# pcubillos/pyratbay

Measured on AMD Instinct MI355X. Metric: spectra/sec (1e5 wavenumbers x 80 layers), higher is better.
Workload: dtype f64; 1 GPU; 1e5 wavenumbers x 80 layers, 1e5 synthetic lines, transit; nwave=100001, nlayers=80, nlines=100000, wnosamp=180, voigt_grid=nlor=100 ndop=50 extent=300 cutoff=25, voigt_table_bytes=1448022784, parallelism=single GPU, 2 independent spectra in flight on 2 HIP streams, ranks=1, priming_spectra_in_init=32

## Files before the change

### pyratbay_amd/csrc/pb_ext_gather.hip

```cpp
#include <algorithm>
#include <climits>
#include <cmath>
#include <type_traits>
#include <vector>

#include "pb_ext_plan.h"

using namespace pbx;

namespace {

template <int RS, int NW>
__global__ __launch_bounds__(NW * 64) void k_ext_resample(LblArgs a)
{
    constexpr int NT = NW * 64;
    constexpr int kTileRS = (NW / RS) * kWaveSpan;
    static_assert(NW % RS == 0, "wavefronts must divide evenly into record shares");
    __shared__ double s_k[NT];
    __shared__ unsigned s_off[NT];
    __shared__ unsigned s_win[NT];

    int tile, layer;
    decode_block(a, tile, layer);
    if (layer < 0 || (a.res_cap > 0 && a.ls_resident[layer]))
        return;
    if (a.tsplit && a.tsplit[((int64_t)tile * kTileRS) / a.ts_tile] != 0)
        return;
    const int row = blockIdx.y;
    const int lane = threadIdx.x & 63;
    const int wave = __builtin_amdgcn_readfirstlane(threadIdx.x >> 6);

    const int64_t t0 = a.wbegin + (int64_t)tile * kTileRS;
    const int64_t tend = min(t0 + kTileRS, a.wbegin + a.wcount);
    const int part = wave % RS;
    const int rlo = (wave / RS) * kWaveSpan;
    const int64_t recbase = (int64_t)layer * a.ngroups;
    const int rhi = (int)min((int64_t)rlo + kWaveSpan, tend - t0);

    const int ofactor = a.ls_ofactor[layer];
    const double kthresh =
        a.ethresh * __longlong_as_double((long long)a.kmax_bits[(int64_t)layer * a.nrows + row]);
    const int osamp = a.osamp;

    double acc[kChunks][kLaneSamples];
#pragma unroll
    for (int s = 0; s < kChunks; s++)
        acc[s][0] = acc[s][1] = 0.0;

    for (int iso = 0; iso < a.niso; iso++) {
        const int iext = a.isoiext[iso];
        if (iext < 0 || (a.add ? 0 : iext) != row)
            continue;
        const int64_t li = (int64_t)layer * a.niso + iso;
        const int ilor = a.li_ilor[li];
        const double alphad = a.li_alphad[li];
        const double dens = a.li_dens[li];
        int64_t reach = a.li_hmax[li];
        if (a.cutoff > 0.0)
            reach = min(reach, (int64_t)(a.cutoff / a.ownstep) + 2 * (int64_t)ofactor + 2);
        reach += osamp + ofactor;
        const int64_t seg0 = a.iso_gstart[iso], seg1 = a.iso_gstart[iso + 1];
        const int64_t g0 = lower_bound_i32(a.giown, seg0, seg1, t0 * osamp - reach);
        const int64_t g1 = lower_bound_i32(a.giown, seg0, seg1, (tend - 1) * osamp + reach + 1);
        if (g0 >= g1)
            continue;
        const double vmin = a.own0 + ((double)a.giown[g0] - 1.0) * a.ownstep;
        const int idop_lo = pb::nearest_index(a.doppler, alphad * vmin, 0, a.ndop - 1);
        const int64_t cell_lo = (int64_t)ilor * a.ndop + idop_lo;
        const int64_t base_idx = a.pm_base[cell_lo] - kTile;
        const double *base = a.pm + base_idx;

        for (int64_t gb = g0; gb < g1; gb += NT) {
            __syncthreads();
            {
                const int64_t g = gb + threadIdx.x;
                double k = 0.0;
                unsigned off = 0, win = 0;
                if (g < g1) {
                    int ulo, uhi, cell, phi, q;
                    if (a.tsplit) {
                        const Rec16 r = a.rec16[(int64_t)layer * a.rec_pitch + a.pos2ph[g]];
                        k = r.k;
                        ulo = r.ulo;
                        uhi = ulo + (int)(r.lc & 0xfffu);
                        cell = (int)(r.lc >> 12);
                        const int d = a.psize[cell] - a.giown[g];
                        q = floor_div_inv(d, a.inv_osamp);
                        phi = d - q * osamp;
                    } else {
                        const int64_t idx = recbase + g;
                        k = a.rec_k[idx];
                        ulo = a.rec_ulo[idx];
                        uhi = a.rec_uhi[idx];
                        cell = a.rec_cell[idx];
                        phi = a.rec_phi[idx];
                        q = a.rec_q[idx];
                    }
                    const int64_t lo = max((int64_t)ulo, t0);
                    const int64_t hi = min((int64_t)uhi, tend);
                    if (!(k < kthresh) && lo < hi) {
                        if (a.add)
                            k *= dens;
                        win = (unsigned)(lo - t0) | ((unsigned)(hi - t0) << 16);
                        off = (unsigned)(a.pm_base[cell] + (int64_t)phi * a.pm_stride[cell] + q +
                                         t0 - base_idx);
                        if (a.experiment == 1)
                            off = (unsigned)(kTile + (lo - t0));
                    } else {
                        k = 0.0;
                    }
                }
                s_k[threadIdx.x] = k;
                s_off[threadIdx.x] = off;
                s_win[threadIdx.x] = win;
            }
            __syncthreads();
            const int nrec = a.experiment == 2 ? 0 : (int)min((int64_t)NT, g1 - gb);
            for (int b = 0; b < nrec; b += 64) {
                const int e = (b + lane) & (NT - 1);
                const unsigned my_win = s_win[e];
                const bool mine = RS == 1 || (int)(((gb + b + lane) >> 6) & (RS - 1)) == part;
                const bool hit = mine && b + lane < nrec && (int)(my_win & 0xffff) < rhi &&
                                 (int)(my_win >> 16) > rlo;
                unsigned long long mask = __ballot(hit);
                const double my_k = s_k[e];
                const unsigned my_off = s_off[e];
                while (mask) {
                    int src[kRecs];
#pragma unroll
                    for (int r = 0; r < kRecs; r++) {
                        src[r] = mask ? __builtin_amdgcn_readfirstlane(__builtin_ctzll(mask))
                                      : -1;
                        mask &= mask - 1;
                    }
                    double2 v[kRecs][kChunks];
                    double kk[kRecs];
                    int lo[kRecs], hi[kRecs];
#pragma unroll
                    for (int r = 0; r < kRecs; r++) {
                        const int sl = src[r] < 0 ? src[0] : src[r];
                        kk[r] = bcast(my_k, sl);
                        const unsigned win = (unsigned)__builtin_amdgcn_readlane((int)my_win, sl);
                        const unsigned off = (unsigned)__builtin_amdgcn_readlane((int)my_off, sl);
                        lo[r] = (int)(win & 0xffff);
                        hi[r] = (int)(win >> 16);
                        if (src[r] < 0)
                            kk[r] = 0.0;
                        const double *tab = base + off;
#pragma unroll
                        for (int s = 0; s < kChunks; s++) {
                            const int j = rlo + s * kChunk + 2 * lane;
                            const int jc = min(max(j, lo[r] - 1), hi[r] - 1);
                            v[r][s] = *reinterpret_cast<const double2 *>(tab + jc);
                        }
                    }
#pragma unroll
                    for (int r = 0; r < kRecs; r++) {
                        const unsigned span = (unsigned)(hi[r] - lo[r]);
#pragma unroll
                        for (int s = 0; s < kChunks; s++) {
                            const int j = rlo + s * kChunk + 2 * lane;
                            acc[s][0] = fma((unsigned)(j - lo[r]) < span ? kk[r] : 0.0,
                                            v[r][s].x, acc[s][0]);
                            acc[s][1] = fma((unsigned)(j + 1 - lo[r]) < span ? kk[r] : 0.0,
                                            v[r][s].y, acc[s][1]);
                        }
                    }
                }
            }
        }
    }

    if (RS > 1) {
        __shared__ double s_acc[NT * kChunks * kLaneSamples];
        __syncthreads();
#pragma unroll
        for (int s = 0; s < kChunks; s++) {
            s_acc[(threadIdx.x * kChunks + s) * kLaneSamples + 0] = acc[s][0];
            s_acc[(threadIdx.x * kChunks + s) * kLaneSamples + 1] = acc[s][1];
        }
        __syncthreads();
        if (part != 0)
            return;
#pragma unroll
        for (int s = 0; s < kChunks; s++) {
            for (int q = 1; q < RS; q++) {
                const int t = threadIdx.x + q * 64;
                acc[s][0] += s_acc[(t * kChunks + s) * kLaneSamples + 0];
                acc[s][1] += s_acc[(t * kChunks + s) * kLaneSamples + 1];
            }
        }
    }
    double *dst = a.ext + ((int64_t)layer * a.nrows + row) * a.wcount + (t0 - a.wbegin);
#pragma unroll
    for (int s = 0; s < kChunks; s++) {
        const int j = rlo + s * kChunk + 2 * lane;
        if (j < rhi)
            dst[j] = acc[s][0];
        if (j + 1 < rhi)
            dst[j + 1] = acc[s][1];
    }
}


template <int NW, int S, bool kDma, int kProbe = 0, int kIssue = 0, int kRows = 1>
__global__ __launch_bounds__(NW * 64, 8) void k_ext_staged(LblArgs a)
{
    constexpr int kThreads = NW * 64;
    constexpr int kSub = NW * kStageSpan;
    constexpr int kT = S * kSub;
    constexpr int kRowRegs = (kStageRowMax + kThreads - 1) / kThreads;
    static_assert(kT < 65536, "window coordinates are packed in 16 bits");
    extern __shared__ __align__(16) unsigned char smem[];
    const int osamp = a.osamp;
    double *s_row = reinterpret_cast<double *>(smem);
    struct __align__(16) Rec {
        double k;
        int qoff;
        unsigned win;
    };
    const int rowspan = a.rowlds + kStagePad;
    constexpr int kNB = 2;
    Rec *s_rec = reinterpret_cast<Rec *>(s_row + kNB * rowspan + kStagePad);
    long long *s_src = reinterpret_cast<long long *>(s_rec + kThreads);
    unsigned long long *s_desc = reinterpret_cast<unsigned long long *>(s_src);
    unsigned long long *s_segmask =
        reinterpret_cast<unsigned long long *>(s_src + kThreads);
    unsigned *s_m = reinterpret_cast<unsigned *>(s_segmask + NW);
    unsigned *s_seg = s_m;
    long long *s_cbase = reinterpret_cast<long long *>(s_m + kThreads);
    int *s_csize = reinterpret_cast<int *>(s_cbase + a.ndop);
    int *s_cstride = s_csize + a.ndop;
    int *s_part = s_cstride + a.ndop;
    const int vmax = osamp * a.nch_max;
    int *s_cum = s_part + NW;
    int *s_phs = s_cum + (vmax + 1);

    int tile, layer, zsplit;
    {
        const int id = blockIdx.x;
        const int k = id >> 3;
        tile = k % a.ntiles;
        const int grp = k / a.ntiles;
        const int unit = grp * 8 + ((grp & 1) ? 7 - (id & 7) : (id & 7));
        if (a.unit_tab) {
            const int e = unit < a.nunits ? a.unit_tab[unit] : -1;
            layer = e < 0 ? -1 : e >> 8;
            zsplit = e & 0xff;
        } else {
            layer = a.nlayers - 1 - unit / a.nsplit;
            zsplit = unit % a.nsplit;
        }
    }
    if (layer < 0 || (a.res_cap > 0 && a.ls_resident[layer]) || (a.wave_cap > 0 && a.ls_wave[layer]))
        return;
    const int nsp = a.tsplit ? a.tsplit[tile] : a.lsplit ? a.lsplit[layer] : a.nsplit;
    if (zsplit >= nsp)
        return;
    const int row = blockIdx.y;
    const int tid = threadIdx.x;
    const int lane = tid & 63;
    const int wave = __builtin_amdgcn_readfirstlane(tid >> 6);
    unsigned long long pc[22] = {0, 0, 0, 0, 0, 0, 0, 0, 0, 0, 0, 0, 0, 0, 0, 0, 0, 0, 0, 0, 0, 0};
    auto tick = [&]() -> unsigned long long {
        if constexpr (kProbe == 4)
            return (unsigned long long)__builtin_amdgcn_s_memtime();
        return 0ull;
    };
    unsigned long long real_birth = 0;
    if constexpr (kProbe == 4) {
        real_birth = (unsigned long long)__builtin_amdgcn_s_memrealtime();
        const unsigned long long c0 = tick();
        const unsigned long long c1 = tick();
        const unsigned long long c2 = tick();
        pc[16] = (c2 - c0) + 0 * c1;
        pc[17] = 1;
    }
    const unsigned long long t_birth = tick();

    const int64_t t0 = a.wbegin + (int64_t)tile * kT;
    const int64_t tend = min(t0 + kT, a.wbegin + a.wcount);
    const int tlen = (int)(tend - t0);
    const int rlo = wave * kStageSpan;

    const double kthresh =
        a.ethresh * __longlong_as_double((long long)a.kmax_bits[(int64_t)layer * a.nrows + row]);
    const int64_t recbase = a.rec16 ? (int64_t)layer * a.rec_pitch - a.grp_lo
                                    : (int64_t)layer * a.ngroups;
    double *const out = zsplit == 0
                            ? a.ext
                            : a.part + (int64_t)(zsplit - 1) * a.nlayers * a.nrows * a.wcount;
    double *const dst = out + ((int64_t)layer * a.nrows + row) * a.wcount + (t0 - a.wbegin);

    double acc[S][4];
#pragma unroll
    for (int u = 0; u < S; u++)
        acc[u][0] = acc[u][1] = acc[u][2] = acc[u][3] = 0.0;
    if (a.accumulate) {
#pragma unroll
        for (int u = 0; u < S; u++)
#pragma unroll
            for (int c = 0; c < 4; c++) {
                const int j = rlo + u * kSub + c * 64 + lane;
                if (j < tlen)
                    acc[u][c] = dst[j];
            }
    }
    for (int i = tid; i < kNB * rowspan + kStagePad; i += kThreads)
        s_row[i] = 0.0;

    double ring[kDma ? 1 : 2 * kRowRegs];
    int rowlim = a.rowlds;
    constexpr bool kMulti = kDma && kIssue == 0 && kRows > 1;
    int pitch = rowspan, nrow = 1;
    static_assert(kRows <= kStageRowsMax && kStageRowsMax <= NW,
                  "a wavefront requests at most one row of a step");
    const unsigned row_lds0 = (unsigned)(size_t)(__attribute__((address_space(3))) char *)(
        reinterpret_cast<char *>(s_row + kStagePad));
    int npiece = (rowlim + 127) >> 7;
    typedef int dma_v4i __attribute__((ext_vector_type(4)));
#define PB_DMA_OPEN "s_mov_b32 %0, m0\n\ts_mov_b32 m0, %1\n\ts_nop 0\n\t"
#define PB_DMA_LD(off) "buffer_load_dwordx4 %2, %3, 0 offen offset:" #off " lds\n\t"
#define PB_DMA_LD1 PB_DMA_LD(0)
#define PB_DMA_LD2 PB_DMA_LD1 PB_DMA_LD(1024)
#define PB_DMA_LD3 PB_DMA_LD2 PB_DMA_LD(2048)
#define PB_DMA_LD4 PB_DMA_LD3 PB_DMA_LD(3072)
#define PB_DMA_GROUP(pad, loads, dst_, voff_)                                                    \
    do {                                                                                         \
        unsigned keep;                                                                           \
        asm volatile(pad PB_DMA_OPEN loads "s_mov_b32 m0, %0"                                    \
                     : "=&s"(keep)                                                               \
                     : "s"(dst_), "v"(voff_), "s"(rsrc)                                          \
                     : "memory");                                                                \
    } while (0)
    auto dma_pieces = [&](unsigned dst, int voff, dma_v4i rsrc) {
        const unsigned dst4 = dst + 4096;
        const int voff4 = voff + 4096;
        switch (npiece) {
        case 1: PB_DMA_GROUP("s_nop 4\n\t", PB_DMA_LD1, dst, voff); break;
        case 2: PB_DMA_GROUP("s_nop 4\n\t", PB_DMA_LD2, dst, voff); break;
        case 3: PB_DMA_GROUP("s_nop 4\n\t", PB_DMA_LD3, dst, voff); break;
        case 4: PB_DMA_GROUP("s_nop 4\n\t", PB_DMA_LD4, dst, voff); break;
        case 5:
            PB_DMA_GROUP("s_nop 4\n\t", PB_DMA_LD4, dst, voff);
            PB_DMA_GROUP("", PB_DMA_LD1, dst4, voff4);
            break;
        case 6:
            PB_DMA_GROUP("s_nop 4\n\t", PB_DMA_LD4, dst, voff);
            PB_DMA_GROUP("", PB_DMA_LD2, dst4, voff4);
            break;
        case 7:
            PB_DMA_GROUP("s_nop 4\n\t", PB_DMA_LD4, dst, voff);
            PB_DMA_GROUP("", PB_DMA_LD3, dst4, voff4);
            break;
        case 8:
            PB_DMA_GROUP("s_nop 4\n\t", PB_DMA_LD4, dst, voff);
            PB_DMA_GROUP("", PB_DMA_LD4, dst4, voff4);
            break;
        default: break;
        }
    };
#undef PB_DMA_GROUP
#undef PB_DMA_LD4
#undef PB_DMA_LD3
#undef PB_DMA_LD2
#undef PB_DMA_LD1
#undef PB_DMA_LD
#undef PB_DMA_OPEN
    auto dma_desc = [&](unsigned long long d, int buf, auto part, int c_lo, int c_hi,
                        unsigned long long tref = 0) {
        const unsigned dlo = (unsigned)__builtin_amdgcn_readfirstlane((int)d);
        const unsigned dhi = (unsigned)__builtin_amdgcn_readfirstlane((int)(d >> 32));
        const long long first = ((long long)(dhi & 0xffu) << 32) | dlo;
        const int len = (int)((dhi >> 8) & 0xfffu), mlo = (int)(dhi >> 20);
        const unsigned long long base = (unsigned long long)(a.pm + first);
        dma_v4i rsrc;
        rsrc.x = __builtin_amdgcn_readfirstlane((int)base);
        rsrc.y = __builtin_amdgcn_readfirstlane((int)((base >> 32) & 0xffffu));
        rsrc.z = __builtin_amdgcn_readfirstlane(len * 8);
        rsrc.w = 0x00020000;
        int voff = (2 * lane - (mlo & ~1)) * 8;
        unsigned dst = (unsigned)__builtin_amdgcn_readfirstlane((int)(row_lds0 + buf * (kMulti ? pitch : rowspan) * 8));
        if constexpr (kProbe == 4) {
            if (tref)
                pc[20] += tick() - tref;
        }
        if constexpr (!decltype(part)::value) {
            dma_pieces(dst, voff, rsrc);
        } else {
            voff += 1024 * c_lo;
            dst += 1024 * (unsigned)c_lo;
            for (int c = c_lo; c < c_hi && c * 128 < rowlim; c++) {
                unsigned keep;
                asm volatile("s_nop 4\n\t"
                             "s_mov_b32 %0, m0\n\t"
                             "s_mov_b32 m0, %1\n\t"
                             "s_nop 0\n\t"
                             "buffer_load_dwordx4 %2, %3, 0 offen lds\n\t"
                             "s_mov_b32 m0, %0"
                             : "=&s"(keep)
                             : "s"(dst), "v"(voff), "s"(rsrc)
                             : "memory");
                voff += 1024;
                dst += 1024;
            }
        }
    };
    auto dma_row = [&](int sg, int buf, unsigned long long tref = 0) {
        dma_desc(s_desc[sg], buf, std::false_type(), 0, 0, tref);
    };
    auto load_row = [&](int sg, auto Rc, double *reg) {
        constexpr int R = decltype(Rc)::value;
        const unsigned long long d = s_desc[sg];
        const unsigned dlo = (unsigned)__builtin_amdgcn_readfirstlane((int)d);
        const unsigned dhi = (unsigned)__builtin_amdgcn_readfirstlane((int)(d >> 32));
        const long long first = ((long long)(dhi & 0xffu) << 32) | dlo;
        const int len = (int)((dhi >> 8) & 0xfffu), mlo = (int)(dhi >> 20);
        const __amdgpu_buffer_rsrc_t rsrc = __builtin_amdgcn_make_buffer_rsrc(
            (void *)(a.pm + first), 0, len * 8, 0x00020000);
        typedef int v2i __attribute__((ext_vector_type(2)));
#pragma unroll
        for (int r = 0; r < R; r++) {
            const v2i v = __builtin_amdgcn_raw_buffer_load_b64(
                rsrc, (tid + r * kThreads - mlo) * 8, 0, 0);
            reg[r] = __hiloint2double(v.y, v.x);
        }
    };
    auto store_row = [&](int buf, auto Rc, const double *reg, auto Dc) {
        constexpr int R = decltype(Rc)::value;
        constexpr int kInFlight = (decltype(Dc)::value - 1) * R;
        __builtin_amdgcn_s_waitcnt((kInFlight & 0xf) | (0x7 << 4) | (0xf << 8) |
                                   ((kInFlight >> 4) << 14));
        double *dst = s_row + kStagePad + buf * rowspan;
#pragma unroll
        for (int r = 0; r < R; r++) {
            if (wave * 64 + r * kThreads >= rowlim)
                continue;
            const int mm = tid + r * kThreads;
            if (mm < a.rowlds)
                dst[mm] = reg[r];
        }
    };

    pc[14] += tick() - t_birth;
    for (int iso = 0; iso < a.niso; iso++) {
        const int iext = a.isoiext[iso];
        if (iext < 0 || (a.add ? 0 : iext) != row)
            continue;
        if ((iso + 1) * osamp <= a.key_lo || iso * osamp >= a.key_hi)
            continue;
        const unsigned long long t_iso = tick();
        const int64_t li = (int64_t)layer * a.niso + iso;
        const double dens = a.li_dens[li];
        int64_t reach = a.li_hmax[li];
        if (a.cutoff > 0.0)
            reach = min(reach, (int64_t)(a.cutoff / a.ownstep) + 2 * (int64_t)a.ls_ofactor[layer] + 2);
        reach += osamp + a.ls_ofactor[layer];
        const int64_t flo = t0 * osamp - reach, fhi = (tend - 1) * osamp + reach;

        __syncthreads();
        const int cell0 = a.li_ilor[li] * a.ndop;
        for (int d = tid; d < a.ndop; d += kThreads) {
            s_cbase[d] = a.pm_base[cell0 + d];
            s_csize[d] = a.psize[cell0 + d];
            s_cstride[d] = a.pm_stride[cell0 + d];
        }
        {
            const int lim = min(a.rowlds, a.li_rowmax[li]);
            if (lim != rowlim) {
                for (int i = tid; i < kNB * rowspan + kStagePad; i += kThreads)
                    s_row[i] = 0.0;
                rowlim = lim;
                npiece = (lim + 127) >> 7;
                if constexpr (kMulti) {
                    const StageSlots sl = stage_slots(a.rowlds, lim, min(kRows, a.rows_cap));
                    pitch = sl.pitch;
                    nrow = sl.rows;
                }
            }
        }
        const int nch = a.nch_max > 1
                            ? (min(a.rowcap, a.li_rowmax[li]) + kChunkRow - 1) / kChunkRow
                            : 1;
        const int nvirt = osamp * nch;
        const int per = (nvirt + kThreads - 1) / kThreads;
        int mine = 0;
        for (int r = 0; r < per; r++) {
            const int pv = tid * per + r;
            const int p = pv / nch, c = pv - p * nch;
            if (pv < nvirt && ((nsp > 1 && p * nsp / osamp != zsplit) ||
                               iso * osamp + p < a.key_lo || iso * osamp + p >= a.key_hi)) {
                s_phs[pv] = 0;
                s_cum[pv] = 0;
            } else if (pv < nvirt) {
                const int32_t *bin = a.ph_bin + ((int64_t)iso * osamp + p) * (a.ph_nbins + 1);
                const int64_t binw = (int64_t)kBinSamples * osamp;
                int64_t clo = flo, chi = fhi;
                if (a.nch_max > 1) {
                    const int64_t c0 = (int64_t)c * kChunkRow;
                    clo = max(clo, (t0 - c0 - kChunkRow - 1) * osamp + a.li_hlo[li]);
                    chi = min(chi, (tend - c0 + 1) * osamp + a.li_hhi[li]);
                    if (chi < clo)
                        chi = clo - 1;
                }
                const int b0 = (int)min((int64_t)a.ph_nbins - 1, max((int64_t)0, clo) / binw);
                const int b1 = (int)min((int64_t)a.ph_nbins - 1, max((int64_t)0, chi + 1) / binw);
                const int32_t l0 = bin[b0], h0 = bin[b0 + 1], l1 = bin[b1], h1 = bin[b1 + 1];
                int64_t s0, s1;
                lower_bound2_i32(a.ph_iown, l0, h0, clo, l1, h1, chi + 1, s0, s1);
                s_phs[pv] = (int)s0;
                s_cum[pv] = (int)(s1 - s0);
                mine += (int)(s1 - s0);
            }
        }
        int incl = mine;
#pragma unroll
        for (int d = 1; d < 64; d <<= 1) {
            const int up = __shfl_up(incl, d);
            if (lane >= d)
                incl += up;
        }
        if (lane == 63)
            s_part[wave] = incl;
        __syncthreads();
        int base = 0, total = 0;
        for (int w = 0; w < NW; w++) {
            const int pw = s_part[w];
            if (w < wave)
                base += pw;
            total += pw;
        }
        int run = base + incl - mine;
        for (int r = 0; r < per; r++) {
            const int pv = tid * per + r;
            if (pv < nvirt) {
                const int c = s_cum[pv];
                s_cum[pv] = run;
                run += c;
            }
        }
        if (tid == 0)
            s_cum[nvirt] = total;
        __syncthreads();
        pc[0] += tick() - t_iso;

        for (int x0 = 0; x0 < total; x0 += kThreads) {
            const int nrec = min(kThreads, total - x0);
            const unsigned long long t_batch = tick();
            pc[11] += 1;
            __syncthreads();
            long long src = -1;
            unsigned mwin = 0;
            {
                double k = 0.0;
                unsigned win = 0;
                int qoff = 0;
                const int x = x0 + tid;
                if (x < total) {
                    int plo = 0, pup = nvirt;
                    while (pup - plo > 1) {
                        const int mid = (plo + pup) >> 1;
                        if (s_cum[mid] <= x)
                            plo = mid;
                        else
                            pup = mid;
                    }
                    const int64_t entry = s_phs[plo] + (x - s_cum[plo]);
                    const int64_t gidx = entry;
                    int c0 = 0;
                    if (a.nch_max > 1)
                        c0 = (plo % nch) * kChunkRow;
                    const int64_t idx = recbase + entry;
                    int ulo, uhi, q, cell, phi;
                    if (a.rec16) {
                        const Rec16 r = a.rec16[idx];
                        k = r.k;
                        ulo = r.ulo;
                        const int lbits = a.nch_max > 1 ? kLongLenBits : 12;
                        uhi = ulo + (int)(r.lc & ((1u << lbits) - 1u));
                        cell = (int)(r.lc >> lbits);
                        const int d = s_csize[cell - cell0] - a.ph_iown[gidx];
                        q = floor_div_inv(d, a.inv_osamp);
                        phi = d - q * osamp;
                        if (a.nch_max > 1) {
                            const int wlo = max(ulo + q, c0), whi = min(uhi + q, c0 + kChunkRow);
                            if (whi > wlo) {
                                ulo = wlo - q;
                                uhi = whi - q;
                            } else {
                                uhi = ulo;
                            }
                        }
                        q -= c0;
                    } else {
                        k = a.rec_k[idx];
                        ulo = a.rec_ulo[idx];
                        uhi = a.rec_uhi[idx];
                        q = a.rec_q[idx];
                        cell = a.rec_cell[idx];
                        phi = a.rec_phi[idx];
                    }
                    const int lo = (int)(max((int64_t)ulo, t0) - t0);
                    const int hi = (int)(min((int64_t)uhi, tend) - t0);
                    if (!(k < kthresh) && lo < hi) {
                        if (a.add)
                            k *= dens;
                        win = (unsigned)lo | ((unsigned)hi << 16);
                        qoff = (int)(q + t0) * 8;
                        if (kDma)
                            qoff -= ((ulo + q) & 1) * 8;
                        src = s_cbase[cell - cell0] + (long long)phi * s_cstride[cell - cell0] + c0;
                        mwin = (unsigned)(ulo + q) | ((unsigned)(uhi + q) << 16);
                    } else {
                        k = 0.0;
                    }
                }
                s_rec[tid].k = k;
                s_rec[tid].qoff = qoff;
                s_rec[tid].win = win;
                s_src[tid] = src;
                s_m[tid] = mwin;
            }
            __syncthreads();
            const unsigned long long t_seg = tick();
            pc[1] += t_seg - t_batch;
            bool start = false;
            {
                if (tid < nrec)
                    start = tid == 0 || s_src[tid] != s_src[tid - 1] || s_m[tid] != s_m[tid - 1];
                const unsigned long long m = __ballot(start);
                if (lane == 0)
                    s_segmask[wave] = m;
            }
            const bool live = start && s_src[tid] >= 0;
            const unsigned long long livemask = __ballot(live);
            if (lane == 0)
                s_part[wave] = __builtin_popcountll(livemask);
            __syncthreads();
            int nseg = 0;
            {
                int before = 0;
                for (int w = 0; w < NW; w++) {
                    const int c = s_part[w];
                    if (w < wave)
                        before += c;
                    nseg += c;
                }
                if (live) {
                    int w = tid >> 6;
                    unsigned long long m = s_segmask[w] & ~((2ull << (tid & 63)) - 1ull);
                    int end = nrec;
                    for (;;) {
                        if (m) {
                            end = min(nrec, w * 64 + (int)__builtin_ctzll(m));
                            break;
                        }
                        if (++w >= NW)
                            break;
                        m = s_segmask[w];
                    }
                    const int pos = before + __builtin_popcountll(livemask & ((1ull << lane) - 1ull));
                    s_seg[pos] = (unsigned)tid | ((unsigned)end << 16);
                    const unsigned long long mlo = mwin & 0xffffu, mhi = mwin >> 16;
                    s_desc[pos] = (unsigned long long)(src + (long long)mlo) | ((mhi - mlo) << 40) |
                                  (mlo << 52);
                }
            }
            __syncthreads();
            pc[2] += tick() - t_seg;
            if (nseg == 0)
                continue;
            unsigned hits[S];
            auto find_hits = [&](int sg0) {
                const int sgl = sg0 + lane;
                const unsigned sd = sgl < nseg ? s_seg[sgl] : 0u;
                const int i0 = (int)(sd & 0xffff), i1 = (int)(sd >> 16);
#pragma unroll
                for (int u = 0; u < S; u++) {
                    const int slo = rlo + u * kSub;
                    int lo = i0, hi = i1;
                    while (lo < hi) {
                        const int mid = (lo + hi) >> 1;
                        if ((int)(s_rec[mid].win >> 16) > slo)
                            hi = mid;
                        else
                            lo = mid + 1;
                    }
                    const int first = lo;
                    hi = i1;
                    while (lo < hi) {
                        const int mid = (lo + hi) >> 1;
                        if ((int)(s_rec[mid].win & 0xffff) >= slo + kStageSpan)
                            hi = mid;
                        else
                            lo = mid + 1;
                    }
                    hits[u] = slo < tlen ? (unsigned)first | ((unsigned)(lo - first) << 16) : 0u;
                }
            };
            auto walk = [&](int sg, int buf) {
                if ((sg & 63) == 0) {
                    const unsigned long long tf = tick();
                    find_hits(sg);
                    pc[3] += tick() - tf;
                }
                bool any = false;
                const char *rowp = reinterpret_cast<const char *>(
                    s_row + kStagePad + buf * (kMulti ? pitch : rowspan) + rlo + lane);
#pragma unroll
                for (int u = 0; u < S; u++) {
                    const unsigned h = (unsigned)__builtin_amdgcn_readlane((int)hits[u], sg & 63);
                    if (h < 0x10000u)
                        continue;
                    if constexpr (kProbe == 4) {
                        pc[12] += h >> 16;
                        any = true;
                    }
                    const int first = (int)(h & 0xffff);
                    const int last = first + (int)(h >> 16);
                    const char *rs = rowp + (size_t)u * kSub * 8;
                    const double2 *recs = reinterpret_cast<const double2 *>(s_rec);
                    auto visit = [&](const double2 raw) {
                        const double k = raw.x;
                        const int qoff = __double2loint(raw.y);
                        if constexpr (kProbe == 1 || kProbe == 2) {
                            const char *base = reinterpret_cast<const char *>(s_row);
                            const int off = ((int)(rs - base) + (kProbe == 1 ? 3 : 1) * 8 * lane + qoff) & ~15;
                            const double2 v0 = *reinterpret_cast<const double2 *>(base + off);
                            const double2 v1 = *reinterpret_cast<const double2 *>(
                                base + off + (kProbe == 1 ? 16 : 1024));
                            acc[u][0] = fma(k, v0.x, acc[u][0]);
                            acc[u][1] = fma(k, v0.y, acc[u][1]);
                            acc[u][2] = fma(k, v1.x, acc[u][2]);
                            acc[u][3] = fma(k, v1.y, acc[u][3]);
                            return;
                        }
                        const double *p0 = reinterpret_cast<const double *>(rs + qoff);
                        const double a0 = p0[0], a1 = p0[64], a2 = p0[128], a3 = p0[192];
                        acc[u][0] = fma(k, a0, acc[u][0]);
                        acc[u][1] = fma(k, a1, acc[u][1]);
                        acc[u][2] = fma(k, a2, acc[u][2]);
                        acc[u][3] = fma(k, a3, acc[u][3]);
                    };
                    int r = first;
                    for (; r + 3 < last; r += 4) {
                        const double2 w0 = recs[r], w1 = recs[r + 1], w2 = recs[r + 2],
                                      w3 = recs[r + 3];
                        visit(w0);
                        visit(w1);
                        visit(w2);
                        visit(w3);
                    }
                    if constexpr (kProbe == 3) {
                        if (r < last) {
                            double2 cur = recs[r];
                            for (; r + 1 < last; r++) {
                                const double2 nxt = recs[r + 1];
                                visit(cur);
                                cur = nxt;
                            }
                            visit(cur);
                        }
                    } else {
                        for (; r < last; r++)
                            visit(recs[r]);
                    }
                }
                if constexpr (kProbe == 4)
                    pc[13] += any ? 1 : 0;
            };
            auto run = [&](auto Dc, auto Rc) {
                constexpr int D = decltype(Dc)::value, R = decltype(Rc)::value;
                static_assert(D == 2, "two register sets, two LDS buffers");
                load_row(0, Rc, ring);
                load_row(min(1, nseg - 1), Rc, ring + R);
                store_row(0, Rc, ring, Dc);
                __syncthreads();
                int sg = 0;
                for (; sg + 2 < nseg; sg += 2) {
                    load_row(sg + 2, Rc, ring);
                    walk(sg, 0);
                    store_row(1, Rc, ring + R, Dc);
                    __syncthreads();
                    load_row(min(sg + 3, nseg - 1), Rc, ring + R);
                    walk(sg + 1, 1);
                    store_row(0, Rc, ring, Dc);
                    __syncthreads();
                }
                walk(sg, 0);
                if (sg + 1 < nseg) {
                    store_row(1, Rc, ring + R, std::integral_constant<int, 1>());
                    __syncthreads();
                    walk(sg + 1, 1);
                }
            };
            if (kDma) {
                if constexpr (kIssue == 1) {
                    unsigned long long dn = s_desc[min(nseg - 1, wave == 0 ? NW : wave)];
                    if (wave == 0)
                        dma_row(0, 0);
                    __builtin_amdgcn_s_waitcnt(0x0f70);
                    __syncthreads();
                    for (int sg = 0; sg < nseg; sg++) {
                        if (sg + 1 < nseg && wave == ((sg + 1) & (NW - 1))) {
                            dma_desc(dn, (sg + 1) & 1, std::false_type(), 0, 0);
                            dn = s_desc[min(nseg - 1, sg + 1 + NW)];
                        }
                        walk(sg, sg & 1);
                        __builtin_amdgcn_s_waitcnt(0x0f70);
                        __syncthreads();
                    }
                    continue;
                }
                if constexpr (kIssue == 2) {
                    constexpr int kPer = (8 + NW - 1) / NW;
                    unsigned long long dn = s_desc[min(nseg - 1, 1)];
                    dma_desc(s_desc[0], 0, std::true_type(), wave * kPer, wave * kPer + kPer);
                    __builtin_amdgcn_s_waitcnt(0x0f70);
                    __syncthreads();
                    for (int sg = 0; sg < nseg; sg++) {
                        const unsigned long long dcur = dn;
                        dn = s_desc[min(nseg - 1, sg + 2)];
                        if (sg + 1 < nseg)
                            dma_desc(dcur, (sg + 1) & 1, std::true_type(), wave * kPer, wave * kPer + kPer);
                        walk(sg, sg & 1);
                        __builtin_amdgcn_s_waitcnt(0x0f70);
                        __syncthreads();
                    }
                    continue;
                }
                if constexpr (!kMulti) {
                    unsigned long long ta = tick();
                    if (wave == 0)
                        dma_row(0, 0);
                    __builtin_amdgcn_s_waitcnt(0x0f70);
                    __syncthreads();
                    if constexpr (kProbe == 4) {
                        const unsigned long long tb = tick();
                        pc[8] += tb - ta;
                        ta = tb;
                    }
                    for (int sg = 0; sg < nseg; sg++) {
                        if (sg + 1 < nseg && wave == ((sg + 1) & (NW - 1)))
                            dma_row(sg + 1, (sg + 1) & 1, ta);
                        if constexpr (kProbe == 4) {
                            const unsigned long long tb = tick();
                            if (sg + 1 < nseg && wave == ((sg + 1) & (NW - 1))) {
                                pc[4] += tb - ta;
                                pc[19] += 1;
                            } else {
                                pc[18] += tb - ta;
                            }
                            ta = tb;
                            const unsigned long long f0 = pc[3];
                            walk(sg, sg & 1);
                            const unsigned long long tc = tick();
                            pc[5] += (tc - ta) - (pc[3] - f0);
                            __builtin_amdgcn_s_waitcnt(0x0f70);
                            const unsigned long long td = tick();
                            pc[6] += td - tc;
                            __syncthreads();
                            ta = tick();
                            pc[7] += ta - td;
                            pc[10] += 1;
                            pc[21] += 1;
                            continue;
                        }
                        walk(sg, sg & 1);
                        __builtin_amdgcn_s_waitcnt(0x0f70);
                        __syncthreads();
                    }
                    continue;
                }
                auto step_end = [&](int s0) { return min(min(s0 + nrow, nseg), (s0 | 63) + 1); };
                auto request = [&](int s0, int s1, int slot0, unsigned long long tref) {
                    const int g = s0 + ((wave - s0) & (NW - 1));
                    if (g < s1)
                        dma_row(g, slot0 + (g - s0), tref);
                    return g < s1;
                };
                unsigned long long ta = tick();
                int sg = 0, se = step_end(0), half = 0;
                request(0, se, 0, 0);
                __builtin_amdgcn_s_waitcnt(0x0f70);
                __syncthreads();
                if constexpr (kProbe == 4) {
                    const unsigned long long tb = tick();
                    pc[8] += tb - ta;
                    ta = tb;
                }
                while (sg < nseg) {
                    const int sn = step_end(se);
                    const bool asked = request(se, sn, (half ^ 1) * nrow, ta);
                    if constexpr (kProbe == 4) {
                        const unsigned long long tb = tick();
                        if (asked) {
                            pc[4] += tb - ta;
                            pc[19] += 1;
                        } else {
                            pc[18] += tb - ta;
                        }
                        ta = tb;
                        const unsigned long long f0 = pc[3];
                        for (int g = sg; g < se; g++)
                            walk(g, half * nrow + (g - sg));
                        const unsigned long long tc = tick();
                        pc[5] += (tc - ta) - (pc[3] - f0);
                        __builtin_amdgcn_s_waitcnt(0x0f70);
                        const unsigned long long td = tick();
                        pc[6] += td - tc;
                        __syncthreads();
                        ta = tick();
                        pc[7] += ta - td;
                        pc[10] += 1;
                        pc[21] += (unsigned long long)(se - sg);
                    } else {
                        (void)asked;
                        for (int g = sg; g < se; g++)
                            walk(g, half * nrow + (g - sg));
                        __builtin_amdgcn_s_waitcnt(0x0f70);
                        __syncthreads();
                    }
                    sg = se;
                    se = sn;
                    half ^= 1;
                }
            } else if (nseg > 0) {
                run(std::integral_constant<int, 2>(), std::integral_constant<int, kRowRegs>());
            }
        }
    }

    const unsigned long long t_out = tick();
#pragma unroll
    for (int u = 0; u < S; u++) {
#pragma unroll
        for (int c = 0; c < 4; c++) {
            const int j = rlo + u * kSub + c * 64 + lane;
            if (j < tlen)
                dst[j] = acc[u][c];
        }
    }
    if constexpr (kProbe == 4) {
        const unsigned long long t_end = tick();
        pc[14] += t_end - t_out;
        pc[9] = t_end - t_birth;
        pc[15] = (unsigned long long)__builtin_amdgcn_s_memrealtime() - real_birth;
        if (lane == 0 && a.probe)
            for (int i = 0; i < 22; i++)
                atomicAdd(&a.probe[(int64_t)layer * 24 + i], pc[i]);
    }
}

__global__ __launch_bounds__(kResThreads) void k_ext_resident(LblArgs a)
{
    extern __shared__ __align__(16) unsigned char smem[];
    struct __align__(16) Rec {
        double k;
        int off;
        unsigned win;
    };
    double *s_prof = reinterpret_cast<double *>(smem);
    const int zslot = a.res_cap;
    Rec *s_rec = reinterpret_cast<Rec *>(s_prof + a.res_cap + 2);
    int *s_cell = reinterpret_cast<int *>(s_rec + kResThreads);
    int *s_part = s_cell + kResThreads;

    int tile, layer;
    decode_block(a, tile, layer);
    if (layer < 0 || !a.ls_resident[layer])
        return;
    const int row = blockIdx.y;
    const int tid = threadIdx.x;
    const int lane = tid & 63;
    const int wave = __builtin_amdgcn_readfirstlane(tid >> 6);

    const int64_t t0 = a.wbegin + (int64_t)tile * kResTile;
    const int64_t tend = min(t0 + kResTile, a.wbegin + a.wcount);
    const int tlen = (int)(tend - t0);
    const double kthresh =
        a.ethresh * __longlong_as_double((long long)a.kmax_bits[(int64_t)layer * a.nrows + row]);
    const int64_t recbase = (int64_t)layer * a.ngroups;
    const int osamp = a.osamp;
    const int ofactor = a.ls_ofactor[layer];

    double acc[kResStrips];
#pragma unroll
    for (int u = 0; u < kResStrips; u++)
        acc[u] = 0.0;
    if (tid == 0)
        s_prof[zslot] = 0.0;

    for (int iso = 0; iso < a.niso; iso++) {
        const int iext = a.isoiext[iso];
        if (iext < 0 || (a.add ? 0 : iext) != row)
            continue;
        const int64_t li = (int64_t)layer * a.niso + iso;
        const double dens = a.li_dens[li];
        int64_t reach = a.li_hmax[li];
        if (a.cutoff > 0.0)
            reach = min(reach, (int64_t)(a.cutoff / a.ownstep) + 2 * (int64_t)ofactor + 2);
        reach += osamp + ofactor;
        const int64_t rs = reach / osamp + 1;
        const int32_t *gs = a.gs_start + (int64_t)iso * (a.nwave + 1);
        const int64_t g0 = gs[max((int64_t)0, t0 - rs)];
        const int64_t g1 = gs[min((int64_t)a.nwave, tend + rs)];

        for (int64_t gb = g0; gb < g1; gb += kResThreads) {
            const int nrec = (int)min((int64_t)kResThreads, g1 - gb);
            __syncthreads();
            {
                double k = 0.0;
                unsigned win = 0;
                int off = 0, cell = -1;
                if (tid < nrec) {
                    const int64_t idx = recbase + gb + tid;
                    k = a.rec_k[idx];
                    const int ulo = a.rec_ulo[idx], uhi = a.rec_uhi[idx];
                    const int lo = (int)(max((int64_t)ulo, t0) - t0);
                    const int hi = (int)(min((int64_t)uhi, tend) - t0);
                    if (!(k < kthresh) && lo < hi) {
                        if (a.add)
                            k *= dens;
                        cell = a.rec_cell[idx];
                        win = (unsigned)lo | ((unsigned)(hi - lo) << 16);
                        off = 8 * (a.rec_phi[idx] * a.pm_stride[cell] + (int)(a.rec_q[idx] + t0));
                    } else {
                        k = 0.0;
                    }
                }
                s_rec[tid].k = k;
                s_rec[tid].off = off;
                s_rec[tid].win = win;
                s_cell[tid] = cell;
            }
            int cur = -1;
            for (;;) {
                __syncthreads();
                int c = s_cell[tid];
                c = c > cur ? c : INT_MAX;
#pragma unroll
                for (int d = 32; d >= 1; d >>= 1)
                    c = min(c, __shfl_xor(c, d));
                if (lane == 0)
                    s_part[wave] = c;
                __syncthreads();
                c = INT_MAX;
                for (int w = 0; w < kResWaves; w++)
                    c = min(c, s_part[w]);
                if (c == INT_MAX)
                    break;
                cur = c;
                {
                    const int n = a.pm_stride[cur] * osamp;
                    const double *src = a.pm + a.pm_base[cur];
                    for (int i = tid; i < n; i += kResThreads)
                        s_prof[i] = src[i];
                }
                __syncthreads();
                const double2 *recs = reinterpret_cast<const double2 *>(s_rec);
#pragma unroll
                for (int u = 0; u < kResStrips; u++) {
                    const int slo = (wave + u * kResWaves) * 64;
                    if (slo >= tlen)
                        continue;
                    int first = INT_MAX, last = -1;
                    for (int b = 0; b < nrec; b += 64) {
                        const int e = b + lane;
                        const unsigned w = s_rec[e].win;
                        const int wlo = (int)(w & 0xffff);
                        const bool hit = s_cell[e] == cur && wlo < slo + 64 &&
                                         wlo + (int)(w >> 16) > slo;
                        const unsigned long long m = __ballot(hit);
                        if (m) {
                            first = min(first, b + (int)__builtin_ctzll(m));
                            last = max(last, b + 63 - (int)__builtin_clzll(m));
                        }
                    }
                    first = __builtin_amdgcn_readfirstlane(first);
                    last = __builtin_amdgcn_readfirstlane(last);
                    const unsigned j = (unsigned)(slo + lane);
                    typedef __attribute__((address_space(3))) const double lds_double;
                    const unsigned prof0 = (unsigned)(uintptr_t)(
                        (__attribute__((address_space(3))) const char *)s_prof);
                    const unsigned j8 = prof0 + j * 8u, z8 = prof0 + (unsigned)zslot * 8u;
                    double sum = acc[u];
#pragma unroll 4
                    for (int r = first; r <= last; r++) {
                        const double2 raw = recs[r];
                        const unsigned w = (unsigned)__double2hiint(raw.y);
                        const bool in = j - (w & 0xffffu) < (w >> 16);
                        const unsigned at = in ? j8 + (unsigned)__double2loint(raw.y) : z8;
                        sum = fma(raw.x, *(lds_double *)(uintptr_t)at, sum);
                    }
                    acc[u] = sum;
                }
            }
        }
    }

    double *dst = a.ext + ((int64_t)layer * a.nrows + row) * a.wcount + (t0 - a.wbegin);
#pragma unroll
    for (int u = 0; u < kResStrips; u++) {
        const int j = (wave + u * kResWaves) * 64 + lane;
        if (j < tlen)
            dst[j] = acc[u];
    }
}

#ifdef PB_EXPERIMENTS
constexpr int kScatterPad = 64;

template <int C>
__device__ inline void scatter_walk(const LblArgs &a, double *s_tile, int layer, int row,
                                    int64_t t0, int64_t tend, double kthresh)
{
    typedef int v2i __attribute__((ext_vector_type(2)));
    typedef int v4i __attribute__((ext_vector_type(4)));
    const int lane = threadIdx.x;
    const int osamp = a.osamp;
    const int ofactor = a.ls_ofactor[layer];
    const Rec32 *recs = a.rec32 + (int64_t)layer * a.ngroups;

    for (int iso = 0; iso < a.niso; iso++) {
        const int iext = a.isoiext[iso];
        if (iext < 0 || (a.add ? 0 : iext) != row)
            continue;
        const int64_t li = (int64_t)layer * a.niso + iso;
        const double dens = a.add ? a.li_dens[li] : 1.0;
        int64_t reach = a.li_hmax[li];
        if (a.cutoff > 0.0)
            reach = min(reach, (int64_t)(a.cutoff / a.ownstep) + 2 * (int64_t)ofactor + 2);
        reach += osamp + ofactor;
        const int64_t rs = reach / osamp + 1;
        const int32_t *gs = a.gs_start + (int64_t)iso * (a.nwave + 1);
        const int g0 = gs[max((int64_t)0, t0 - rs)];
        const int g1 = gs[min((int64_t)a.nwave, tend + rs)];

        v4i w0 = {0, 0, 0, 0}, w1 = {0, 0, 0, 0};
        auto fetch = [&](int g) {
            const v4i *p = reinterpret_cast<const v4i *>(recs + min(g + lane, g1 - 1));
            w0 = p[0];
            w1 = p[1];
        };
        if (g0 < g1)
            fetch(g0);
        for (int gb = g0; gb < g1; gb += 64) {
            const double kk = __hiloint2double(w0.y, w0.x);
            const long long off = ((long long)w0.w << 32) | (unsigned)w0.z;
            const int lo = max(w1.x, (int)t0), hi = min(w1.y, (int)tend);
            const bool ok = gb + lane < g1 && !(kk < kthresh) && lo < hi;
            const double b_k = kk * dens;
            const long long b_src = off + lo;
            const int b_lo = lo - (int)t0, b_n = hi - lo;
            unsigned long long live = __ballot(ok);
            if (gb + 64 < g1)
                fetch(gb + 64);

            struct Cur {
                int dst, nch;
                double k;
            };
            auto start = [&](double (&v)[C], Cur &c) {
                const int sl = (int)__builtin_ctzll(live);
                live &= live - 1;
                c.k = bcast(b_k, sl);
                const int s_lo = __builtin_amdgcn_readlane((int)b_src, sl);
                const int s_hi = __builtin_amdgcn_readlane((int)(b_src >> 32), sl);
                const int n = __builtin_amdgcn_readlane(b_n, sl);
                c.dst = __builtin_amdgcn_readlane(b_lo, sl);
                c.nch = (n + 63) >> 6;
                const __amdgpu_buffer_rsrc_t rsrc = __builtin_amdgcn_make_buffer_rsrc(
                    (void *)(a.pm + (((long long)s_hi << 32) | (unsigned)s_lo)), 0, n * 8,
                    0x00020000);
#pragma unroll
                for (int q = 0; q < C; q++) {
                    const v2i w = __builtin_amdgcn_raw_buffer_load_b64(rsrc, lane * 8, q * 512, 0);
                    v[q] = __hiloint2double(w.y, w.x);
                }
            };
            auto finish = [&](const double (&v)[C], const Cur &c) {
                double *dst = s_tile + c.dst + lane;
#pragma unroll
                for (int q = 0; q < C; q++)
                    if (q < c.nch)
                        __hip_atomic_fetch_add(dst + q * 64, c.k * v[q], __ATOMIC_RELAXED,
                                               __HIP_MEMORY_SCOPE_WORKGROUP);
            };
            double va[C], vb[C];
            Cur ca, cb;
            if (!live)
                continue;
            start(va, ca);
            for (;;) {
                if (!live) {
                    finish(va, ca);
                    break;
                }
                start(vb, cb);
                finish(va, ca);
                if (!live) {
                    finish(vb, cb);
                    break;
                }
                start(va, ca);
                finish(vb, cb);
            }
        }
    }
}

template <int T>
__global__ __launch_bounds__(64) void k_ext_scatter(LblArgs a)
{
    __shared__ double s_tile[T + kScatterPad];
    int tile, layer;
    decode_block(a, tile, layer);
    if (layer < 0)
        return;
    const int row = blockIdx.y;
    const int lane = threadIdx.x;
    const int64_t t0 = a.wbegin + (int64_t)tile * T;
    const int64_t tend = min(t0 + T, a.wbegin + a.wcount);
    const int tlen = (int)(tend - t0);
    const double kthresh =
        a.ethresh * __longlong_as_double((long long)a.kmax_bits[(int64_t)layer * a.nrows + row]);
    for (int i = lane; i < T + kScatterPad; i += 64)
        s_tile[i] = 0.0;
    const int rowmax = a.ls_block[layer] / a.osamp;
// ... 443 lines not shown
```

Baseline: 1188 spectra/s.

## Precompute LDS record offsets and uniform scalars to trim staged walk loop overhead

The hit word now holds an absolute LDS byte offset plus a count split into a multiple-of-four part and a remainder, so the inner record walk iterates over LDS pointers and handles the tail with fixed 1- and 2-record steps instead of index arithmetic. Buffer offsets are carried as running byte offsets toggled by XOR, and per-wave DMA ownership is tracked with an incrementing counter instead of modulo tests. Several wave-uniform values (threshold, density, cell base, pitch, row count) are forced into scalar registers with readfirstlane. The goal is less VALU/SALU bookkeeping in the hot gather loop, which adds a static limit on the LDS size and more intricate step scheduling.

```diff
diff --git a/pyratbay_amd/csrc/pb_ext_gather.hip b/pyratbay_amd/csrc/pb_ext_gather.hip
--- a/pyratbay_amd/csrc/pb_ext_gather.hip
+++ b/pyratbay_amd/csrc/pb_ext_gather.hip
@@ -222,6 +222,13 @@
     const int rowspan = a.rowlds + kStagePad;
     constexpr int kNB = 2;
     Rec *s_rec = reinterpret_cast<Rec *>(s_row + kNB * rowspan + kStagePad);
+    static_assert((kNB * (kStageRowMax + kStagePad) + kStagePad) * 8 + kThreads * 16 <= 65536,
+                  "a hit word holds the LDS offset of a record in 16 bits");
+    typedef double rec_v2 __attribute__((ext_vector_type(2)));
+    typedef const rec_v2 rec_cv2;
+    typedef __attribute__((address_space(3))) rec_cv2 *rec_lds_p;
+    const unsigned rec_off0 =
+        (unsigned)(size_t)(__attribute__((address_space(3))) char *)(reinterpret_cast<char *>(s_rec));
     long long *s_src = reinterpret_cast<long long *>(s_rec + kThreads);
     unsigned long long *s_desc = reinterpret_cast<unsigned long long *>(s_src);
     unsigned long long *s_segmask =
@@ -283,8 +290,12 @@
     const int tlen = (int)(tend - t0);
     const int rlo = wave * kStageSpan;
 
-    const double kthresh =
-        a.ethresh * __longlong_as_double((long long)a.kmax_bits[(int64_t)layer * a.nrows + row]);
+    auto uniform = [](double x) {
+        return __hiloint2double(__builtin_amdgcn_readfirstlane(__double2hiint(x)),
+                                __builtin_amdgcn_readfirstlane(__double2loint(x)));
+    };
+    const double kthresh = uniform(
+        a.ethresh * __longlong_as_double((long long)a.kmax_bits[(int64_t)layer * a.nrows + row]));
     const int64_t recbase = a.rec16 ? (int64_t)layer * a.rec_pitch - a.grp_lo
                                     : (int64_t)layer * a.ngroups;
     double *const out = zsplit == 0
@@ -367,7 +378,7 @@
 #undef PB_DMA_LD1
 #undef PB_DMA_LD
 #undef PB_DMA_OPEN
-    auto dma_desc = [&](unsigned long long d, int buf, auto part, int c_lo, int c_hi,
+    auto dma_desc = [&](unsigned long long d, unsigned boff, auto part, int c_lo, int c_hi,
                         unsigned long long tref = 0) {
         const unsigned dlo = (unsigned)__builtin_amdgcn_readfirstlane((int)d);
         const unsigned dhi = (unsigned)__builtin_amdgcn_readfirstlane((int)(d >> 32));
@@ -380,7 +391,7 @@
         rsrc.z = __builtin_amdgcn_readfirstlane(len * 8);
         rsrc.w = 0x00020000;
         int voff = (2 * lane - (mlo & ~1)) * 8;
-        unsigned dst = (unsigned)__builtin_amdgcn_readfirstlane((int)(row_lds0 + buf * (kMulti ? pitch : rowspan) * 8));
+        unsigned dst = (unsigned)__builtin_amdgcn_readfirstlane((int)(row_lds0 + boff));
         if constexpr (kProbe == 4) {
             if (tref)
                 pc[20] += tick() - tref;
@@ -406,8 +417,9 @@
             }
         }
     };
-    auto dma_row = [&](int sg, int buf, unsigned long long tref = 0) {
-        dma_desc(s_desc[sg], buf, std::false_type(), 0, 0, tref);
+    auto bufoff = [&](int buf) { return (unsigned)(buf * rowspan * 8); };
+    auto dma_row = [&](int sg, unsigned boff, unsigned long long tref = 0) {
+        dma_desc(s_desc[sg], boff, std::false_type(), 0, 0, tref);
     };
     auto load_row = [&](int sg, auto Rc, double *reg) {
         constexpr int R = decltype(Rc)::value;
@@ -451,7 +463,7 @@
             continue;
         const unsigned long long t_iso = tick();
         const int64_t li = (int64_t)layer * a.niso + iso;
-        const double dens = a.li_dens[li];
+        const double dens = uniform(a.li_dens[li]);
         int64_t reach = a.li_hmax[li];
         if (a.cutoff > 0.0)
             reach = min(reach, (int64_t)(a.cutoff / a.ownstep) + 2 * (int64_t)a.ls_ofactor[layer] + 2);
@@ -459,7 +471,7 @@
         const int64_t flo = t0 * osamp - reach, fhi = (tend - 1) * osamp + reach;
 
         __syncthreads();
-        const int cell0 = a.li_ilor[li] * a.ndop;
+        const int cell0 = __builtin_amdgcn_readfirstlane(a.li_ilor[li] * a.ndop);
         for (int d = tid; d < a.ndop; d += kThreads) {
             s_cbase[d] = a.pm_base[cell0 + d];
             s_csize[d] = a.psize[cell0 + d];
@@ -474,8 +486,8 @@
                 npiece = (lim + 127) >> 7;
                 if constexpr (kMulti) {
                     const StageSlots sl = stage_slots(a.rowlds, lim, min(kRows, a.rows_cap));
-                    pitch = sl.pitch;
-                    nrow = sl.rows;
+                    pitch = __builtin_amdgcn_readfirstlane(sl.pitch);
+                    nrow = __builtin_amdgcn_readfirstlane(sl.rows);
                 }
             }
         }
@@ -695,32 +707,32 @@
                         else
                             lo = mid + 1;
                     }
-                    hits[u] = slo < tlen ? (unsigned)first | ((unsigned)(lo - first) << 16) : 0u;
+                    const unsigned n = (unsigned)(lo - first);
+                    hits[u] = slo < tlen && n
+                                  ? (rec_off0 + (unsigned)first * 16u) << 16 | (n & ~3u) << 4 | (n & 3u)
+                                  : 0u;
                 }
             };
-            auto walk = [&](int sg, int buf) {
-                if ((sg & 63) == 0) {
-                    const unsigned long long tf = tick();
-                    find_hits(sg);
-                    pc[3] += tick() - tf;
-                }
+            auto block_hits = [&](int sg) {
+                const unsigned long long tf = tick();
+                find_hits(sg);
+                pc[3] += tick() - tf;
+            };
+            auto walk_row = [&](int sg, const char *rowp) {
                 bool any = false;
-                const char *rowp = reinterpret_cast<const char *>(
-                    s_row + kStagePad + buf * (kMulti ? pitch : rowspan) + rlo + lane);
 #pragma unroll
                 for (int u = 0; u < S; u++) {
                     const unsigned h = (unsigned)__builtin_amdgcn_readlane((int)hits[u], sg & 63);
-                    if (h < 0x10000u)
+                    if (h == 0u)
                         continue;
                     if constexpr (kProbe == 4) {
-                        pc[12] += h >> 16;
+                        pc[12] += ((h & 0xffc0u) >> 4) + (h & 3u);
                         any = true;
                     }
-                    const int first = (int)(h & 0xffff);
-                    const int last = first + (int)(h >> 16);
                     const char *rs = rowp + (size_t)u * kSub * 8;
-                    const double2 *recs = reinterpret_cast<const double2 *>(s_rec);
-                    auto visit = [&](const double2 raw) {
+                    rec_lds_p recs = (rec_lds_p)(size_t)(h >> 16);
+                    const rec_lds_p trips_end = (rec_lds_p)(size_t)((h >> 16) + (h & 0xffc0u));
+                    auto visit = [&](const rec_v2 raw) {
                         const double k = raw.x;
                         const int qoff = __double2loint(raw.y);
                         if constexpr (kProbe == 1 || kProbe == 2) {
@@ -742,33 +754,45 @@
                         acc[u][2] = fma(k, a2, acc[u][2]);
                         acc[u][3] = fma(k, a3, acc[u][3]);
                     };
-                    int r = first;
-                    for (; r + 3 < last; r += 4) {
-                        const double2 w0 = recs[r], w1 = recs[r + 1], w2 = recs[r + 2],
-                                      w3 = recs[r + 3];
+                    for (; recs != trips_end; recs += 4) {
+                        const rec_v2 w0 = recs[0], w1 = recs[1], w2 = recs[2], w3 = recs[3];
                         visit(w0);
                         visit(w1);
                         visit(w2);
                         visit(w3);
                     }
+                    const int left = (int)(h & 3u);
                     if constexpr (kProbe == 3) {
-                        if (r < last) {
-                            double2 cur = recs[r];
-                            for (; r + 1 < last; r++) {
-                                const double2 nxt = recs[r + 1];
+                        if (left) {
+                            rec_v2 cur = recs[0];
+                            for (int r = 1; r < left; r++) {
+                                const rec_v2 nxt = recs[r];
                                 visit(cur);
                                 cur = nxt;
                             }
                             visit(cur);
                         }
                     } else {
-                        for (; r < last; r++)
-                            visit(recs[r]);
+                        if (left & 1) {
+                            visit(recs[0]);
+                            recs += 1;
+                        }
+                        if (left & 2) {
+                            const rec_v2 w0 = recs[0], w1 = recs[1];
+                            visit(w0);
+                            visit(w1);
+                        }
                     }
                 }
                 if constexpr (kProbe == 4)
                     pc[13] += any ? 1 : 0;
             };
+            auto walk = [&](int sg, int buf) {
+                if ((sg & 63) == 0)
+                    block_hits(sg);
+                walk_row(sg, reinterpret_cast<const char *>(s_row + kStagePad + buf * rowspan + rlo + lane));
+            };
+            (void)walk;
             auto run = [&](auto Dc, auto Rc) {
                 constexpr int D = decltype(Dc)::value, R = decltype(Rc)::value;
                 static_assert(D == 2, "two register sets, two LDS buffers");
@@ -803,7 +827,7 @@
                     __syncthreads();
                     for (int sg = 0; sg < nseg; sg++) {
                         if (sg + 1 < nseg && wave == ((sg + 1) & (NW - 1))) {
-                            dma_desc(dn, (sg + 1) & 1, std::false_type(), 0, 0);
+                            dma_desc(dn, bufoff((sg + 1) & 1), std::false_type(), 0, 0);
                             dn = s_desc[min(nseg - 1, sg + 1 + NW)];
                         }
                         walk(sg, sg & 1);
@@ -822,7 +846,7 @@
                         const unsigned long long dcur = dn;
                         dn = s_desc[min(nseg - 1, sg + 2)];
                         if (sg + 1 < nseg)
-                            dma_desc(dcur, (sg + 1) & 1, std::true_type(), wave * kPer, wave * kPer + kPer);
+                            dma_desc(dcur, bufoff((sg + 1) & 1), std::true_type(), wave * kPer, wave * kPer + kPer);
                         walk(sg, sg & 1);
                         __builtin_amdgcn_s_waitcnt(0x0f70);
                         __syncthreads();
@@ -830,6 +854,10 @@
                     continue;
                 }
                 if constexpr (!kMulti) {
+                    const unsigned flip8 = (unsigned)rowspan * 8u;
+                    const char *const lane_row = reinterpret_cast<const char *>(s_row + kStagePad + rlo + lane);
+                    unsigned cur8 = 0;
+                    int mine = wave == 0 ? NW : wave;
                     unsigned long long ta = tick();
                     if (wave == 0)
                         dma_row(0, 0);
@@ -840,9 +868,12 @@
                         pc[8] += tb - ta;
                         ta = tb;
                     }
-                    for (int sg = 0; sg < nseg; sg++) {
-                        if (sg + 1 < nseg && wave == ((sg + 1) & (NW - 1)))
-                            dma_row(sg + 1, (sg + 1) & 1, ta);
+                    for (int sg = 0; sg < nseg; sg++, cur8 ^= flip8) {
+                        if (mine == sg + 1) {
+                            if (mine < nseg)
+                                dma_row(mine, cur8 ^ flip8, ta);
+                            mine += NW;
+                        }
                         if constexpr (kProbe == 4) {
                             const unsigned long long tb = tick();
                             if (sg + 1 < nseg && wave == ((sg + 1) & (NW - 1))) {
@@ -853,7 +884,9 @@
                             }
                             ta = tb;
                             const unsigned long long f0 = pc[3];
-                            walk(sg, sg & 1);
+                            if ((sg & 63) == 0)
+                                block_hits(sg);
+                            walk_row(sg, lane_row + cur8);
                             const unsigned long long tc = tick();
                             pc[5] += (tc - ta) - (pc[3] - f0);
                             __builtin_amdgcn_s_waitcnt(0x0f70);
@@ -866,21 +899,42 @@
                             pc[21] += 1;
                             continue;
                         }
-                        walk(sg, sg & 1);
+                        if ((sg & 63) == 0)
+                            block_hits(sg);
+                        walk_row(sg, lane_row + cur8);
                         __builtin_amdgcn_s_waitcnt(0x0f70);
                         __syncthreads();
                     }
                     continue;
                 }
-                auto step_end = [&](int s0) { return min(min(s0 + nrow, nseg), (s0 | 63) + 1); };
-                auto request = [&](int s0, int s1, int slot0, unsigned long long tref) {
-                    const int g = s0 + ((wave - s0) & (NW - 1));
-                    if (g < s1)
-                        dma_row(g, slot0 + (g - s0), tref);
-                    return g < s1;
+                constexpr bool kAligned = kRows <= 2;
+                const unsigned pitch8 = (unsigned)pitch * 8u, flip8 = (unsigned)nrow * pitch8;
+                const char *const lane_row = reinterpret_cast<const char *>(s_row + kStagePad + rlo + lane);
+                int mine = wave;
+                auto request = [&](int s0, int s1, unsigned boff0, unsigned long long tref) {
+                    const bool ask = mine < s1;
+                    if (ask) {
+                        dma_row(mine, boff0 + (unsigned)(mine - s0) * pitch8, tref);
+                        mine += NW;
+                    }
+                    return ask;
                 };
                 unsigned long long ta = tick();
-                int sg = 0, se = step_end(0), half = 0;
+                int bend = kAligned ? nseg : min(64, nseg);
+                int sg = 0, se = min(nrow, bend), hits_from = 0;
+                unsigned cur8 = 0;
+                auto walk_step = [&]() {
+                    if (sg == hits_from) {
+                        block_hits(sg);
+                        hits_from += 64;
+                    }
+                    const char *rp = lane_row + cur8;
+                    int g = sg;
+                    do {
+                        walk_row(g, rp);
+                        rp += pitch8;
+                    } while (++g < se);
+                };
                 request(0, se, 0, 0);
                 __builtin_amdgcn_s_waitcnt(0x0f70);
                 __syncthreads();
@@ -889,9 +943,13 @@
                     pc[8] += tb - ta;
                     ta = tb;
                 }
-                while (sg < nseg) {
-                    const int sn = step_end(se);
-                    const bool asked = request(se, sn, (half ^ 1) * nrow, ta);
+                do {
+                    if constexpr (!kAligned) {
+                        if (se == bend)
+                            bend = min(bend + 64, nseg);
+                    }
+                    const int sn = min(se + nrow, bend);
+                    const bool asked = request(se, sn, cur8 ^ flip8, ta);
                     if constexpr (kProbe == 4) {
                         const unsigned long long tb = tick();
                         if (asked) {
@@ -902,8 +960,7 @@
                         }
                         ta = tb;
                         const unsigned long long f0 = pc[3];
-                        for (int g = sg; g < se; g++)
-                            walk(g, half * nrow + (g - sg));
+                        walk_step();
                         const unsigned long long tc = tick();
                         pc[5] += (tc - ta) - (pc[3] - f0);
                         __builtin_amdgcn_s_waitcnt(0x0f70);
@@ -916,15 +973,14 @@
                         pc[21] += (unsigned long long)(se - sg);
                     } else {
                         (void)asked;
-                        for (int g = sg; g < se; g++)
-                            walk(g, half * nrow + (g - sg));
+                        walk_step();
                         __builtin_amdgcn_s_waitcnt(0x0f70);
                         __syncthreads();
                     }
                     sg = se;
                     se = sn;
-                    half ^= 1;
-                }
+                    cur8 ^= flip8;
+                } while (sg < nseg);
             } else if (nseg > 0) {
                 run(std::integral_constant<int, 2>(), std::integral_constant<int, kRowRegs>());
             }
```

Result: faster. 1266 spectra/s (median of 6 runs) (+6.6%).
